# ysymyth/3D-SDN

Measured on AMD Instinct MI355X. Metric: rendered-objects/sec (FFD decode + transform + silhouette/normal/depth @384, fwd+bwd), higher is better.
Workload: dtype f32

## Files before the change

3d-sdn_amd/csrc/transform.hip:

```cpp
#include "sdn_common.h"

namespace sdn {

struct PtfParams {
    const float* verts;
    const float* scales;
    const float* quat;
    const float* trans;
    const float* persp;
    const float* zoom_to;
    const float* zoom_fixed;
    float* out;
    float* zooms;
    unsigned long long* key;
    int n, V;
};

__device__ __forceinline__ void quat_matrix(const float* q, float T[9])
{
    const float a = q[0], b = q[1], c = q[2], d = q[3];
    T[0] = ((a * a + b * b) - c * c) - d * d;
    T[1] = 2 * b * c - 2 * a * d;
    T[2] = 2 * b * d + 2 * a * c;
    T[3] = 2 * b * c + 2 * a * d;
// ... 42 lines not shown
    if (P.zoom_fixed) return;
#pragma unroll
    for (int o = 32; o > 0; o >>= 1) {
        const unsigned long long other = __shfl_xor(key, o, 64);
        key = other < key ? other : key;
    }
    if ((threadIdx.x & 63) == 0) red[threadIdx.x >> 6] = key;
    __syncthreads();
    if (threadIdx.x == 0) {
        unsigned long long k = red[0];
        for (int i = 1; i < 4; i++) k = red[i] < k ? red[i] : k;
        P.key[P.n + (size_t)b * gridDim.x + blockIdx.x] = k;
    }
}

__global__ __launch_bounds__(256) void k_ptf_fwd_b(const PtfParams P)
{
    __shared__ unsigned long long red[4];
    const int b = blockIdx.y;
    const int v = blockIdx.x * 256 + threadIdx.x;
    unsigned long long key = ~0ull;
    for (unsigned i = threadIdx.x; i < gridDim.x; i += 256) {
        const unsigned long long k = P.key[P.n + (size_t)b * gridDim.x + i];
        key = k < key ? k : key;
    }
#pragma unroll
    for (int o = 32; o > 0; o >>= 1) {
        const unsigned long long other = __shfl_xor(key, o, 64);
        key = other < key ? other : key;
    }
    if ((threadIdx.x & 63) == 0) red[threadIdx.x >> 6] = key;
    __syncthreads();
    key = red[0];
    for (int i = 1; i < 4; i++) key = red[i] < key ? red[i] : key;
    if (v >= P.V) return;
    const float zoom = __uint_as_float((unsigned)(key >> 32)) * P.zoom_to[b];
    float* o = P.out + ((size_t)b * P.V + v) * 3;
    o[2] = o[2] / zoom;
    if (v == 0) {
        P.zooms[b] = zoom;
        P.key[b] = key;
    }
}

struct PtfBwdParams {
    PtfParams f;
    const float* out;
    const float* g_out;
    const float* g_zooms;
    float* g_verts;
    float* acc;
    float* g_scales;
    float* g_quat;
    float* g_trans;
    float* g_persp;
    float* g_zoom_to;
    int s_parts;
};

__global__ __launch_bounds__(256) void k_ptf_bwd_a(const PtfBwdParams B)
{
    __shared__ float red[4];
    const int b = blockIdx.y, V = B.f.V;
    float s = 0.f;
    for (int v = blockIdx.x * 256 + threadIdx.x; v < V; v += gridDim.x * 256) {
        const size_t i = ((size_t)b * V + v) * 3 + 2;
        s += B.g_out[i] * B.out[i];
    }
#pragma unroll
    for (int o = 32; o > 0; o >>= 1) s += __shfl_xor(s, o, 64);
    if ((threadIdx.x & 63) == 0) red[threadIdx.x >> 6] = s;
    __syncthreads();
    if (threadIdx.x == 0) B.acc[20 * (size_t)B.f.n + 16 * b + blockIdx.x] = ((red[0] + red[1]) + red[2]) + red[3];
    if (blockIdx.x == 0 && threadIdx.x < 20) B.acc[20 * b + threadIdx.x] = 0.f;
}

__device__ __forceinline__ float ptf_S(const PtfBwdParams& B, int b, int nparts)
{
    float s = 0.f;
    for (int i = 0; i < nparts; i++) s += B.acc[20 * (size_t)B.f.n + 16 * b + i];
    return s;
}

__global__ __launch_bounds__(256) void k_ptf_bwd_b(const PtfBwdParams B)
{
    __shared__ float red[4][18];
    const int b = blockIdx.y, V = B.f.V;
    const int v = blockIdx.x * 256 + threadIdx.x;
    float part[18];
#pragma unroll
    for (int k = 0; k < 18; k++) part[k] = 0.f;
    if (v < V) {
        float T[9];
        quat_matrix(B.f.quat + 4 * b, T);
        const float* sc = B.f.scales + 3 * b;
        const float* p0 = B.f.persp + 3 * b;
        const unsigned long long key = B.f.key[b];
        const float rmin = __uint_as_float((unsigned)(key >> 32));
        const int vstar = (int)(unsigned)(key & 0xffffffffull);
        const float zoom = rmin * B.f.zoom_to[b];
        float dzoom = -ptf_S(B, b, B.s_parts) / zoom;
        if (B.g_zooms) dzoom += B.g_zooms[b];
        const size_t i = ((size_t)b * V + v) * 3;
        const float X = B.out[i], Y = B.out[i + 1], Z = B.out[i + 2] * zoom;
        float gX = B.g_out[i], gY = B.g_out[i + 1], gZ = B.g_out[i + 2] / zoom;
        if (v == vstar) {
            const float dr = dzoom * B.f.zoom_to[b];
            const float ax = fabsf(X), ay = fabsf(Y);
            const float m = fmaxf(ax, ay);
            gZ += dr * (Z >= 0.f ? 1.f : -1.f) / m;
            const float dm = -dr * fabsf(Z) / (m * m);
            if (ax >= ay)
                gX += dm * (X >= 0.f ? 1.f : -1.f);
            else
                gY += dm * (Y >= 0.f ? 1.f : -1.f);
        }
        const float kx = p0[0] / p0[2], ky = p0[1] / p0[2];
        const float gw0 = gX, gw1 = gY, gw2 = (gZ - kx * gX) - ky * gY;
        part[3] = -gX * Z / p0[2];
        part[4] = -gY * Z / p0[2];
        part[5] = (gX * p0[0] + gY * p0[1]) * Z / (p0[2] * p0[2]);
        part[0] = gw0;
        part[1] = gw1;
        part[2] = gw2;
        const float* vin = B.f.verts + i;
        const float u0 = vin[0] * sc[0], u1 = vin[1] * sc[1], u2 = vin[2] * sc[2];
        part[6] = gw0 * u0;
        part[7] = gw0 * u1;
        part[8] = gw0 * u2;
        part[9] = gw1 * u0;
        part[10] = gw1 * u1;
        part[11] = gw1 * u2;
        part[12] = gw2 * u0;
        part[13] = gw2 * u1;
        part[14] = gw2 * u2;
        const float gu0 = (T[0] * gw0 + T[3] * gw1) + T[6] * gw2;
        const float gu1 = (T[1] * gw0 + T[4] * gw1) + T[7] * gw2;
        const float gu2 = (T[2] * gw0 + T[5] * gw1) + T[8] * gw2;
        part[15] = gu0 * vin[0];
        part[16] = gu1 * vin[1];
        part[17] = gu2 * vin[2];
        float* gv = B.g_verts + i;
        gv[0] = gu0 * sc[0];
        gv[1] = gu1 * sc[1];
        gv[2] = gu2 * sc[2];
    }
#pragma unroll
    for (int k = 0; k < 18; k++) {
        float s = part[k];
#pragma unroll
        for (int o = 32; o > 0; o >>= 1) s += __shfl_xor(s, o, 64);
        if ((threadIdx.x & 63) == 0) red[threadIdx.x >> 6][k] = s;
    }
    __syncthreads();
    if (threadIdx.x < 18)
        unsafeAtomicAdd(B.acc + 20 * b + threadIdx.x,
                        ((red[0][threadIdx.x] + red[1][threadIdx.x]) + red[2][threadIdx.x]) + red[3][threadIdx.x]);
}

__global__ void k_ptf_bwd_c(const PtfBwdParams B)
{
    const int b = blockIdx.x * blockDim.x + threadIdx.x;
    if (b >= B.f.n) return;
    const float* A = B.acc + 20 * b;
    const float* q = B.f.quat + 4 * b;
    const float a = q[0], bq = q[1], c = q[2], d = q[3];
    const float* g = A + 6;
    B.g_quat[4 * b + 0] = 2 * a * ((g[0] + g[4]) + g[8]) + 2 * (((((-d * g[1] + c * g[2]) + d * g[3]) - bq * g[5]) - c * g[6]) + bq * g[7]);
    B.g_quat[4 * b + 1] = 2 * bq * ((g[0] - g[4]) - g[8]) + 2 * (((((c * g[1] + d * g[2]) + c * g[3]) - a * g[5]) + d * g[6]) + a * g[7]);
    B.g_quat[4 * b + 2] = 2 * c * ((-g[0] + g[4]) - g[8]) + 2 * (((((bq * g[1] + a * g[2]) + bq * g[3]) + d * g[5]) - a * g[6]) + d * g[7]);
    B.g_quat[4 * b + 3] = 2 * d * ((-g[0] - g[4]) + g[8]) + 2 * (((((-a * g[1] + bq * g[2]) + a * g[3]) + c * g[5]) + bq * g[6]) + c * g[7]);
    for (int k = 0; k < 3; k++) {
        if (B.g_persp == B.g_trans) {
            B.g_trans[3 * b + k] = A[k] + A[3 + k];
        } else {
            B.g_trans[3 * b + k] = A[k];
            B.g_persp[3 * b + k] = A[3 + k];
        }
        B.g_scales[3 * b + k] = A[15 + k];
    }
    const unsigned long long key = B.f.key[b];
    const float rmin = __uint_as_float((unsigned)(key >> 32));
    const float zoom = rmin * B.f.zoom_to[b];
    float dzoom = -ptf_S(B, b, B.s_parts) / zoom;
    if (B.g_zooms) dzoom += B.g_zooms[b];
    B.g_zoom_to[b] = dzoom * rmin;
}

}

using namespace sdn;

SDN_API int sdn_perspective_transform_scratch(int n, int V, size_t* key_bytes, size_t* acc_bytes)
{
    if (n <= 0 || V <= 0 || (!key_bytes && !acc_bytes))
        return fail(SDN_EINVAL, "sdn_perspective_transform_scratch: bad arguments");
    if (key_bytes) *key_bytes = (size_t)n * (1 + (size_t)cdiv(V, 256)) * sizeof(unsigned long long);
    if (acc_bytes) *acc_bytes = (size_t)n * 36 * sizeof(float);
    return SDN_OK;
}

SDN_API int sdn_perspective_transform(const float* verts, const float* scales, const float* quat, const float* trans,
                                      const float* persp, const float* zoom_to, const float* zoom_fixed, int n, int V,
                                      float* out, float* zooms, void* key, sdnStream stream)
{
    if (!verts || !scales || !quat || !trans || !persp || (!zoom_to && !zoom_fixed) || !out || !zooms || !key || n <= 0 ||
        V <= 0)
        return fail(SDN_EINVAL, "sdn_perspective_transform: bad arguments");
    hipStream_t st = (hipStream_t)stream;
    PtfParams P{verts, scales, quat, trans, persp, zoom_to, zoom_fixed, out, zooms, (unsigned long long*)key, n, V};
    const dim3 grid(cdiv(V, 256), (unsigned)n);
    if (zoom_fixed) {
        hipLaunchKernelGGL(k_ptf_fwd_a, grid, dim3(256), 0, st, P);
        return check_launch("k_ptf_fwd (given zoom)");
    }
    hipLaunchKernelGGL(k_ptf_fwd_a, grid, dim3(256), 0, st, P);
    hipLaunchKernelGGL(k_ptf_fwd_b, grid, dim3(256), 0, st, P);
    return check_launch("k_ptf_fwd");
}

SDN_API int sdn_perspective_transform_bwd(const float* verts, const float* scales, const float* quat, const float* trans,
                                          const float* persp, const float* zoom_to, int n, int V, const float* out,
                                          const void* key, const float* g_out, const float* g_zooms, float* g_verts,
                                          float* g_scales, float* g_quat, float* g_trans, float* g_persp,
                                          float* g_zoom_to, float* acc, sdnStream stream)
{
    if (!verts || !scales || !quat || !trans || !persp || !zoom_to || !out || !key || !g_out || !g_verts || !g_scales ||
        !g_quat || !g_trans || !g_persp || !g_zoom_to || !acc || n <= 0 || V <= 0)
        return fail(SDN_EINVAL, "sdn_perspective_transform_bwd: bad arguments");
    hipStream_t st = (hipStream_t)stream;
    PtfBwdParams B;
    B.f = PtfParams{verts, scales, quat, trans, persp, zoom_to, nullptr, nullptr, nullptr, (unsigned long long*)key, n, V};
    B.out = out;
    B.g_out = g_out;
    B.g_zooms = g_zooms;
    B.g_verts = g_verts;
    B.acc = acc;
    B.g_scales = g_scales;
    B.g_quat = g_quat;
    B.g_trans = g_trans;
    B.g_persp = g_persp;
    B.g_zoom_to = g_zoom_to;
    const unsigned vb = cdiv(V, 256);
    B.s_parts = (int)(vb < 16 ? vb : 16);
    hipLaunchKernelGGL(k_ptf_bwd_a, dim3((unsigned)B.s_parts, (unsigned)n), dim3(256), 0, st, B);
    hipLaunchKernelGGL(k_ptf_bwd_b, dim3(vb, (unsigned)n), dim3(256), 0, st, B);
    hipLaunchKernelGGL(k_ptf_bwd_c, dim3(cdiv(n, 64)), dim3(64), 0, st, B);
    return check_launch("k_ptf_bwd");
}

namespace sdn {

__global__ __launch_bounds__(64) void k_pose_params(const float* __restrict__ theta, const float* __restrict__ log_scales, int n,
                                                    float* __restrict__ quat, float* __restrict__ scales)
{
    const int i = blockIdx.x * 64 + threadIdx.x;
    if (i >= n) return;
    const float h = theta[i] / 2;
    quat[4 * i + 0] = cosf(h);
    quat[4 * i + 1] = 0.f;
    quat[4 * i + 2] = sinf(h);
    quat[4 * i + 3] = 0.f;
#pragma unroll
    for (int d = 0; d < 3; d++) scales[3 * i + d] = expf(log_scales[3 * i + d]);
}

__global__ __launch_bounds__(64) void k_pose_params_bwd(const float* __restrict__ theta, const float* __restrict__ scales,
                                                        const float* __restrict__ g_quat, const float* __restrict__ g_scales, int n,
                                                        float* __restrict__ g_theta, float* __restrict__ g_log_scales)
{
    const int i = blockIdx.x * 64 + threadIdx.x;
    if (i >= n) return;
    if (g_theta) {
        const float h = theta[i] / 2;
        const float a = g_quat ? g_quat[4 * i + 0] : 0.f, c = g_quat ? g_quat[4 * i + 2] : 0.f;
        g_theta[i] = (a * (-sinf(h)) + c * cosf(h)) / 2;
    }
    if (g_log_scales) {
#pragma unroll
        for (int d = 0; d < 3; d++) g_log_scales[3 * i + d] = g_scales ? g_scales[3 * i + d] * scales[3 * i + d] : 0.f;
    }
}

struct PoseAlgebra {
    const float *centre, *extent, *focals, *delta, *log_scales, *log_depths, *t2;
    float *theta, *alpha, *quat, *scales, *depth, *c2, *trans, *persp, *zoom;
    int n, training;
    float image_size, render_size;
};

__device__ __forceinline__ void camera_ray(float row, float col, float r[3], float* norm)
{
    const float l = sqrtf((col * col + row * row) + 1.0f);
    r[0] = col / l;
    r[1] = -row / l;
    r[2] = -1.0f / l;
    *norm = l;
}

__global__ __launch_bounds__(64) void k_pose_algebra(const PoseAlgebra P)
{
    const int i = blockIdx.x * 64 + threadIdx.x;
    if (i >= P.n) return;
    const float d0 = P.delta[2 * i], d1 = P.delta[2 * i + 1];
    const float theta = atan2f(d1, d0);
    P.theta[i] = theta;
    const float h = theta / 2;
    P.quat[4 * i + 0] = cosf(h);
    P.quat[4 * i + 1] = 0.f;
    P.quat[4 * i + 2] = sinf(h);
    P.quat[4 * i + 3] = 0.f;
#pragma unroll
    for (int d = 0; d < 3; d++) P.scales[3 * i + d] = expf(P.log_scales[3 * i + d]);
    const float e0 = P.extent[2 * i], e1 = P.extent[2 * i + 1], c0 = P.centre[2 * i], c1 = P.centre[2 * i + 1];
    const float depth = sqrtf(expf(P.log_depths[i]) / (e0 * e1));
    P.depth[i] = depth;
    const float q0 = c0 + P.t2[2 * i] * e0, q1 = c1 + P.t2[2 * i + 1] * e1;
    P.c2[2 * i] = q0;
    P.c2[2 * i + 1] = q1;
    float r[3], l;
    camera_ray(q0, q1, r, &l);
    const float tx = depth * r[0], ty = depth * r[1], tz = depth * r[2];
    P.trans[3 * i] = tx;
    P.trans[3 * i + 1] = ty;
    P.trans[3 * i + 2] = tz;
    const float a = -(theta - atanf(tx / tz)) + 3.14159265358979323846f;
    const float two_pi = 6.28318530717958647692f;
    float m = fmodf(a, two_pi);
    if (m != 0.f && m < 0.f) m += two_pi;
    P.alpha[i] = m - 3.14159265358979323846f;
// ... 130 lines not shown
```

3d-sdn_amd/csrc/raster_fwd.hip:

```cpp
#include <mutex>
#include <type_traits>
#include <vector>

#include "camera_math.h"
#include "raster_math.h"
#include "sdn_common.h"

namespace sdn {

constexpr int TS = 32;
constexpr int NTHR = (TS / 2) * (TS / 2);
constexpr int NWAVE = NTHR / 64;
static_assert(NTHR % 64 == 0 && NTHR >= 2 * TS && TS <= 32, "tile / workgroup geometry (hit queue packs px, py in 5 bits)");
constexpr int QCAP = 512;
constexpr int FREC = 13;
#ifndef SDN_LAB_SMALL_AREA
#define SDN_LAB_SMALL_AREA 32
#endif
constexpr int SMALL_AREA = SDN_LAB_SMALL_AREA;
#ifndef SDN_LAB_SPAN_AREA
#define SDN_LAB_SPAN_AREA 256
#endif
constexpr int SPAN_AREA = SDN_LAB_SPAN_AREA;
#ifndef SDN_LAB_HIZ_MIN_LIST
#define SDN_LAB_HIZ_MIN_LIST 257
#endif
constexpr int HIZ_MIN_LIST = SDN_LAB_HIZ_MIN_LIST;
#ifndef SDN_K1_HIZ
#define SDN_K1_HIZ 1
#endif
constexpr uint32_t TB_CULLED = 0x000000FFu;

struct FwdParams {
    const float* faces;
    const float* textures;
    const float* bg;
    float* face_inv;
    int32_t* face_index_map;
    float* weight_map;
    float* depth_map;
    float* rgb_map;
    float* rgb_out;
    float* alpha_out;
    float* depth_out;
    const uint32_t* tilebox;
    const uint4* pixbox;
    const uint32_t* tile_off;
    const uint32_t* tile_list;
    const uint32_t* overflow;
    const uint32_t* tile_order;
    const uint32_t* thin_count;
    const float4* thin_list;
    unsigned long long* counters;
    uint32_t list_cap;
    double eps;
    int ts, bs, nf, S, ntx, flags, bg_per_batch;
    int hiz;
    float near_le, far_f;
};

constexpr float THIN_MARGIN = 4.0f;

__device__ __forceinline__ float face_margin_px(const float f[9], int S)
{
    const float ex0 = f[3] - f[0], ey0 = f[4] - f[1];
    const float ex1 = f[6] - f[0], ey1 = f[7] - f[1];
    const float ex2 = f[6] - f[3], ey2 = f[7] - f[4];
    const float l0 = sqrtf(ex0 * ex0 + ey0 * ey0);
    const float l1 = sqrtf(ex1 * ex1 + ey1 * ey1);
    const float l2 = sqrtf(ex2 * ex2 + ey2 * ey2);
    const float lmax = fmaxf(l0, fmaxf(l1, l2));
    const float perim = l0 + l1 + l2;
    float cmax = fmaxf(fmaxf(fabsf(f[0]), fabsf(f[1])), fmaxf(fabsf(f[3]), fabsf(f[4])));
    cmax = fmaxf(cmax, fmaxf(fabsf(f[6]), fabsf(f[7])));
    const float area2 = fabsf(ex0 * ey1 - ex1 * ey0) - 9.5367432e-7f * lmax * lmax;
    if (!(area2 > 0.0f)) return -1.0f;
    const float delta = 9.5367432e-7f * (1.0f + cmax);
    const float base = 0.004f * fmaxf(1.0f, (float)S * (1.0f / 1024.0f)) + 0.5f * (float)S * delta;
    const float m = base + 0.5f * (float)S * (delta * perim * lmax / area2);
    if (!(m < (float)S)) return -1.0f;
    return m;
}

constexpr int HIST_MAX = 4096;

template <bool K1, bool GATHER>
__global__ __launch_bounds__(256) void k_face_setup(const float* __restrict__ faces, int nf, int S, int ntx,
                                                     float* __restrict__ face_inv, uint32_t* __restrict__ tilebox,
                                                     uint4* __restrict__ pixbox, uint32_t* __restrict__ tile_count,
                                                     uint32_t* __restrict__ thin_count, float4* __restrict__ thin_list,
                                                     const FaceSource G)
{
    __shared__ uint32_t hist[HIST_MAX];
    const int ntiles = ntx * ntx;
    const bool use_lds = ntiles <= HIST_MAX;
    if (use_lds)
        for (int t = threadIdx.x; t < ntiles; t += 256) hist[t] = 0u;
    __syncthreads();
    const int b = blockIdx.y;
    const int t_local = blockIdx.x * 256 + threadIdx.x;
    uint32_t* gcount = tile_count + (size_t)b * ntiles;
    const bool pairs = GATHER && G.fill_back != 0;
    const int nthr = pairs ? G.nf0 : nf;
    float v[3][3], pf[9];
    if constexpr (GATHER) {
        if (t_local < nthr) {
// ... 408 lines not shown
#pragma unroll
        for (int dx = 0; dx < 2; dx++) {
            const int dy = 1 - dyi;
            const int px = 2 * qx + dx, py = 2 * qy + dy;
            const int gx = X0 + px, gy = Y0 + py;
            if (gx >= S || gy >= S) continue;
            any_valid = true;
            const PixelResult r = shade_pixel(P, b, zbuf[py * TS + px], gx, gy);
            const size_t q = ((size_t)b * S + gy) * S + gx;
            if (save) {
                P.face_index_map[q] = r.fn;
                P.depth_map[q] = r.zp;
            }
            if (save && !lazy) {
                P.weight_map[q * 3 + 0] = r.w[0];
                P.weight_map[q * 3 + 1] = r.w[1];
                P.weight_map[q * 3 + 2] = r.w[2];
                if (want_rgb) {
                    P.rgb_map[q * 3 + 0] = r.rgb[0];
                    P.rgb_map[q * 3 + 1] = r.rgb[1];
                    P.rgb_map[q * 3 + 2] = r.rgb[2];
                }
            }
            if (aa) {
                s_alpha = s_alpha + r.alpha;
                s_depth = s_depth + r.zp;
#pragma unroll
                for (int k = 0; k < 3; k++) s_rgb[k] = s_rgb[k] + r.rgb[k];
            } else {
                const size_t o = ((size_t)b * S + (S - 1 - gy)) * S + gx;
                if (want_alpha) P.alpha_out[o] = r.alpha;
                if (want_depth) P.depth_out[o] = r.zp;
                if (want_rgb) {
#pragma unroll
                    for (int k = 0; k < 3; k++)
                        P.rgb_out[(((size_t)b * 3 + k) * S + (S - 1 - gy)) * S + gx] = r.rgb[k];
                }
            }
        }
    }
    if (aa && any_valid) {
        const int oc = X0 / 2 + qx;
        const int orow = R - 1 - (Y0 / 2 + qy);
        const size_t o = ((size_t)b * R + orow) * R + oc;
        if (want_alpha) P.alpha_out[o] = s_alpha * 0.25f;
        if (want_depth) P.depth_out[o] = s_depth * 0.25f;
        if (want_rgb) {
#pragma unroll
            for (int k = 0; k < 3; k++) P.rgb_out[(((size_t)b * 3 + k) * R + orow) * R + oc] = s_rgb[k] * 0.25f;
        }
    }
}

__device__ __forceinline__ void hiz_refresh(const uint32_t* zhi, uint32_t* blockmax, const int lane)
{
    uint32_t m[4] = {0u, 0u, 0u, 0u};
#pragma unroll
    for (int i = 0; i < 16; i++) m[i >> 2] = max(m[i >> 2], zhi[2 * (i * 64 + lane) + 1]);
#pragma unroll
    for (int rb = 0; rb < 4; rb++) {
        uint32_t v = m[rb];
        v = max(v, (uint32_t)__shfl_xor((int)v, 1, 64));
        v = max(v, (uint32_t)__shfl_xor((int)v, 2, 64));
        v = max(v, (uint32_t)__shfl_xor((int)v, 4, 64));
        v = max(v, (uint32_t)__shfl_xor((int)v, 32, 64));
        m[rb] = v;
    }
    if ((lane & 39) == 0) {
#pragma unroll
        for (int rb = 0; rb < 4; rb++) blockmax[rb * 4 + (lane >> 3)] = m[rb];
    }
    __builtin_amdgcn_wave_barrier();
}
__device__ __forceinline__ bool hiz_hidden(const uint32_t* blockmax, const uint32_t zc, const int x0, const int x1, const int y0,
                                           const int y1)
{
    uint32_t zb = 0u;
    for (int by = y0 >> 3; by <= (y1 >> 3); by++)
        for (int bx = x0 >> 3; bx <= (x1 >> 3); bx++) zb = max(zb, blockmax[by * (TS / 8) + bx]);
    return zc > zb;
}

template <bool COUNT, int HIZ>
__global__ __launch_bounds__(NTHR) void k_raster_tiles(const FwdParams P)
{
    unsigned n_cand = 0, n_in = 0, n_key = 0;
    unsigned long long c_fetch = 0, c_small = 0, c_large = 0, c_thin = 0, c_epi = 0, t_mark = 0, t_begin = 0;
    auto tick = [&](unsigned long long& acc) {
        if constexpr (COUNT) {
            const unsigned long long now = wall_clock64();
            acc += now - t_mark;
            t_mark = now;
        }
    };
    if constexpr (COUNT) t_begin = t_mark = wall_clock64();
    __shared__ unsigned long long zbuf[TS * TS];
    __shared__ uint32_t q_fn[QCAP];
    __shared__ float xtab[TS], ytab[TS];
    __shared__ uint32_t q_count, next_batch, next_thin;
    __shared__ uint32_t hit_queue[NWAVE][128];
    __shared__ float face_rec[NWAVE][64 * FREC];
    __shared__ uint32_t blockmax[(TS / 8) * (TS / 8)];
    static_assert(TS == 32, "the hi-z refresh maps 64 lanes x 16 reads onto a 32 x 32 tile");

    const int tid = threadIdx.x;
    const int lane = tid & 63, wave = tid >> 6;
    const int ntiles_all = P.ntx * P.ntx;
    const uint32_t gid = P.tile_order[blockIdx.x];
    const int b = (int)(gid / (uint32_t)ntiles_all), tile = (int)(gid % (uint32_t)ntiles_all);
    const int tx = tile % P.ntx, ty = tile / P.ntx;
    const int X0 = tx * TS, Y0 = ty * TS;
    const int S = P.S, nf = P.nf;

    for (int i = tid; i < TS * TS; i += NTHR) zbuf[i] = ~0ull;
    if (tid < TS)
        xtab[tid] = pixel_to_ndc(X0 + tid, S);
    else if (tid < 2 * TS)
        ytab[tid - TS] = pixel_to_ndc(Y0 + tid - TS, S);
    if (tid == 0) q_count = next_batch = next_thin = 0;
    if (tid < (TS / 8) * (TS / 8)) blockmax[tid] = 0xffffffffu;
    __syncthreads();

    const float4* thin_cull = P.thin_list + (size_t)b * nf * 2;
    const uint32_t n_thin = P.thin_count[b];
    const float4 thin_c0 = thin_cull[min(tid, 2 * nf - 1)];
    const uint32_t* tb = P.tilebox + (size_t)b * nf;
    const uint4* pbx = P.pixbox + (size_t)b * nf;
    const float* faces_b = P.faces + (size_t)b * nf * 9;
    const float* finv_b = P.face_inv + (size_t)b * nf * 9;

    auto shade_hit = [&](const float z0, const float z1, const float z2, const float (&inv)[9], const uint32_t qf,
                         const int px, const int py) {
        float bw[3];
        bary_weights(inv, X0 + px, Y0 + py, bw);
        const float zp = persp_depth(bw, z0, z1, z2);
        if (zp > P.near_le && zp < P.far_f) {
            if constexpr (COUNT) n_key++;
            const unsigned long long key = ((unsigned long long)ord_bits(zp) << 32) | qf;
            atomicMin(&zbuf[py * TS + px], key);
        }
    };
    uint32_t* hq = hit_queue[wave];
    float* frec = face_rec[wave];
    int hq_n = 0;
    auto drain = [&](const int count) {
        if (lane < count) {
            const uint32_t e = hq[lane];
            const int slot = (int)(e & 63u), px = (int)((e >> 6) & 31u), py = (int)((e >> 11) & 31u);
            const float* r = frec + slot * FREC;
            float inv[9];
#pragma unroll
            for (int k = 0; k < 9; k++) inv[k] = r[3 + k];
            shade_hit(r[0], r[1], r[2], inv, __float_as_uint(r[12]), px, py);
        }
    };
    const uint32_t* zhi = reinterpret_cast<const uint32_t*>(zbuf);
    auto behind = [&](const uint32_t zc, const int px, const int py) -> bool { return zc > zhi[2 * (py * TS + px) + 1]; };
    bool hiz_on = false;
    auto refresh_hiz = [&]() { hiz_refresh(zhi, blockmax, lane); };
    auto push_hits = [&](const bool hit, const uint32_t entry) {
        const unsigned long long hm = __ballot(hit);
        if (hm) {
            if (hit) hq[hq_n + (int)__popcll(hm & ((1ull << lane) - 1ull))] = entry;
            hq_n += (int)__popcll(hm);
            __builtin_amdgcn_wave_barrier();
            if (hq_n >= 64) {
                drain(64);
                __builtin_amdgcn_wave_barrier();
                const uint32_t rest = (lane < hq_n - 64) ? hq[64 + lane] : 0u;
                __builtin_amdgcn_wave_barrier();
                hq[lane] = rest;
                hq_n -= 64;
                __builtin_amdgcn_wave_barrier();
            }
        }
    };
    auto raster_batch = [&](const uint32_t* ids, const int n) {
        if constexpr (HIZ > 0) {
            if (HIZ == 1 || hiz_on) refresh_hiz();
        }
        const int kshift = 31 - __clz(64 / n);
        const int k = 1 << kshift;
        const int q = lane >> kshift, sub = lane & (k - 1);
        const bool mine = q < n;
        const uint32_t qf_l = mine ? ids[q] : 0u;
        uint4 pb_l = make_uint4(0u, 0u, 0u, 0u);
        float f_l[9], inv_l[9];
#pragma unroll
        for (int kk = 0; kk < 9; kk++) f_l[kk] = inv_l[kk] = 0.0f;
        if (mine) {
            pb_l = pbx[qf_l];
#pragma unroll
            for (int kk = 0; kk < 9; kk++) f_l[kk] = faces_b[(size_t)qf_l * 9 + kk];
#pragma unroll
            for (int kk = 0; kk < 9; kk++) inv_l[kk] = finv_b[(size_t)qf_l * 9 + kk];
        }
        const int lx0 = max((int)(pb_l.x & 0xffffu), X0), lx1 = min((int)(pb_l.x >> 16), X0 + TS - 1);
        const int ly0 = max((int)(pb_l.y & 0xffffu), Y0), ly1 = min((int)(pb_l.y >> 16), Y0 + TS - 1);
        const int lw = lx1 - lx0 + 1, lh = ly1 - ly0 + 1;
        int area_l = (mine && lw > 0 && lh > 0) ? lw * lh : 0;
        const float zmin_l = fminf(f_l[2], fminf(f_l[5], f_l[8]));
        const uint32_t zc_l = (zmin_l > 0.0f) ? ord_bits(zmin_l * 0.99999f) : 0u;
        if constexpr (HIZ > 0) {
            if ((HIZ == 1 || hiz_on) && area_l > 0 && zc_l != 0u && hiz_hidden(blockmax, zc_l, lx0 - X0, lx1 - X0, ly0 - Y0, ly1 - Y0))
                area_l = 0;
        }
        if (mine && sub == 0) {
            float* r = frec + q * FREC;
            r[0] = f_l[2];
            r[1] = f_l[5];
            r[2] = f_l[8];
#pragma unroll
            for (int kk = 0; kk < 9; kk++) r[3 + kk] = inv_l[kk];
            r[12] = __uint_as_float(qf_l);
        }
        __builtin_amdgcn_wave_barrier();
        if constexpr (COUNT) {
            asm volatile("s_waitcnt vmcnt(0) lgkmcnt(0)" ::: "memory");
            tick(c_fetch);
        }
        {
            const bool small = area_l > 0 && area_l <= SMALL_AREA * k;
            const float rw = 1.0f / (float)(lw > 0 ? lw : 1);
            for (int i = sub; __ballot(small && i < area_l) != 0ull; i += k) {
                bool hit = false;
                int px = 0, py = 0;
                if (small && i < area_l) {
                    const int yy = (int)(((float)i + 0.5f) * rw);
                    const int xx = i - yy * lw;
                    px = lx0 - X0 + xx;
                    py = ly0 - Y0 + yy;
                    if constexpr (COUNT) n_cand++;
                    hit = inside_ndc(f_l, xtab[px], ytab[py]);
                    if constexpr (COUNT) n_in += hit ? 1u : 0u;
                    if (hit) hit = !behind(zc_l, px, py);
                }
                push_hits(hit, (uint32_t)q | ((uint32_t)px << 6) | ((uint32_t)py << 11));
            }
        }
        tick(c_small);
        unsigned long long big = __ballot(area_l > SMALL_AREA * k && sub == 0);
        const float fS = (float)S, fS1 = (float)(S - 1);
        while (big) {
            const int j = __builtin_amdgcn_readfirstlane(__ffsll((long long)big) - 1);
            big &= big - 1ull;
            const int x0 = __builtin_amdgcn_readlane(lx0, j), y0 = __builtin_amdgcn_readlane(ly0, j);
            const int w = __builtin_amdgcn_readlane(lw, j), h = __builtin_amdgcn_readlane(lh, j);
            const uint32_t zc = (uint32_t)__builtin_amdgcn_readlane((int)zc_l, j);
            const float mj = __int_as_float(__builtin_amdgcn_readlane((int)pb_l.z, j));
            const uint32_t slot = (uint32_t)(j >> kshift);
            float f[9];
#pragma unroll
            for (int kk = 0; kk < 9; kk++) f[kk] = __int_as_float(__builtin_amdgcn_readlane(__float_as_int(f_l[kk]), j));
            if (w * h <= SPAN_AREA) {
                const int area = w * h;
                const float rw = 1.0f / (float)w;
                for (int i0 = 0; i0 < area; i0 += 64) {
                    const int i = i0 + lane;
                    bool hit = false;
                    int px = 0, py = 0;
                    if (i < area) {
                        const int yy = (int)(((float)i + 0.5f) * rw);
                        const int xx = i - yy * w;
                        px = x0 - X0 + xx;
                        py = y0 - Y0 + yy;
                        if constexpr (COUNT) n_cand++;
                        hit = inside_ndc(f, xtab[px], ytab[py]);
                        if constexpr (COUNT) n_in += hit ? 1u : 0u;
                        if (hit) hit = !behind(zc, px, py);
                    }
                    push_hits(hit, slot | ((uint32_t)px << 6) | ((uint32_t)py << 11));
                }
                continue;
            }
            const int hs = h > 1 ? 32 - __clz(h - 1) : 0;
            const int rshift = 6 - hs, per_row = 1 << rshift;
            const int row = lane >> rshift, rsub = lane & (per_row - 1);
            const bool rvalid = row < h;
            const int py = y0 - Y0 + (rvalid ? row : 0);
            const float yp = ytab[py];
            const int bx0 = x0 - X0;
            float lo = (float)bx0, hi = (float)(bx0 + w - 1);
#pragma unroll
            for (int e = 0; e < 3; e++) {
                const float xa = f[3 * e], ya = f[3 * e + 1], xb = f[(3 * e + 3) % 9], yb = f[(3 * e + 4) % 9];
                const float D = xb - xa, E = yb - ya;
                if (E != 0.0f) {
                    const float rE = __builtin_amdgcn_rcpf(E);
                    const float xe = xa + (yp - ya) * D * rE;
                    const float pe = (xe * fS + fS1) * 0.5f - (float)X0;
                    const float sl = mj * __builtin_amdgcn_sqrtf(D * D + E * E) * fabsf(rE) + 1.0f;
                    if (E > 0.0f)
                        hi = fminf(hi, pe + sl);
                    else
                        lo = fmaxf(lo, pe - sl);
                }
            }
            const int xl = max(bx0, (int)floorf(fminf(lo, 64.0f)));
            const int xr = min(bx0 + w - 1, (int)ceilf(fmaxf(hi, -64.0f)));
            const int len = rvalid ? xr - xl + 1 : 0;
            for (int i = rsub; __ballot(i < len) != 0ull; i += per_row) {
                bool hit = false;
                int px = 0;
                if (i < len) {
                    px = xl + i;
                    if constexpr (COUNT) n_cand++;
                    hit = inside_ndc(f, xtab[px], yp);
                    if constexpr (COUNT) n_in += hit ? 1u : 0u;
                    if (hit) hit = !behind(zc, px, py);
                }
                push_hits(hit, slot | ((uint32_t)px << 6) | ((uint32_t)py << 11));
            }
        }
        if (hq_n) {
            drain(hq_n);
            hq_n = 0;
            __builtin_amdgcn_wave_barrier();
        }
        tick(c_large);
    };

    const float4* thin_recs = thin_cull + nf;
    auto thin_cull_pass = [&]() {
        const float cx = (float)X0 + 0.5f * (float)(TS - 1), cy = (float)Y0 + 0.5f * (float)(TS - 1);
        const float reach = 0.7072f * (float)TS + 0.4f;
#ifndef SDN_LAB_NO_THIN_CULL
        for (uint32_t t = tid; t < n_thin; t += NTHR) {
            const float4 c = t < (uint32_t)NTHR ? thin_c0 : thin_cull[t];
            if (fabsf(cx * c.x + cy * c.y - c.z) > c.w + reach) continue;
            const uint32_t slot = atomicAdd(&q_count, 1u);
            if (slot < (uint32_t)QCAP) q_fn[slot] = t;
        }
#endif
    };
    auto thin_items = [&]() {
#ifndef SDN_LAB_NO_THIN
        const uint32_t queued = q_count;
        const bool all = queued > (uint32_t)QCAP;
        const uint32_t n_loop = all ? n_thin : queued;
        constexpr int ROWS_PER_ITEM = 8, GROUPS = TS / ROWS_PER_ITEM;
        for (;;) {
            uint32_t first = 0;
            if (lane == 0) first = atomicAdd(&next_thin, 64u);
            first = (uint32_t)__builtin_amdgcn_readfirstlane((int)first);
            if (first >= n_loop * GROUPS) break;
            const uint32_t item = first + (uint32_t)lane;
            if (item >= n_loop * GROUPS) continue;
            const uint32_t c = item / GROUPS;
            const int g = (int)(item % GROUPS);
            const uint32_t t = all ? c : q_fn[c];
            const float4 e0 = thin_cull[t], e1 = thin_recs[t];
            const float nx = e0.x, ny = e0.y, band = e0.w, ax = e1.x, ay = e1.y;
            const uint32_t qf = __float_as_uint(e1.z);
            float f[9];
            bool loaded = false;
            for (int py = g * ROWS_PER_ITEM; py < (g + 1) * ROWS_PER_ITEM; py++) {
                const float off = ((float)(Y0 + py) - ay) * ny;
// ... 720 lines not shown
```

Before: 23570.

## Fuse perspective-transform backward finalize into main kernel via last-block ticket

Merges the per-object finalize kernel into the main backward kernel: the last block to arrive for each object, detected with an atomic ticket counter in slot 19 of the accumulator, computes the quaternion, translation, scale and zoom gradients. The main kernel also becomes a grid-stride loop with 1024-thread blocks capped at 16 blocks per object, so each thread accumulates several vertices in registers before one batched shuffle reduction. This removes a kernel launch and cuts the number of atomics, in exchange for release/acquire fence handling and fewer, larger blocks. The ticket counter relies on slot 19 being zeroed by the earlier kernel, which it is.

```diff
diff --git a/3d-sdn_amd/csrc/transform.hip b/3d-sdn_amd/csrc/transform.hip
--- a/3d-sdn_amd/csrc/transform.hip
+++ b/3d-sdn_amd/csrc/transform.hip
@@ -148,87 +148,20 @@
     return s;
 }
 
-__global__ __launch_bounds__(256) void k_ptf_bwd_b(const PtfBwdParams B)
-{
-    __shared__ float red[4][18];
-    const int b = blockIdx.y, V = B.f.V;
-    const int v = blockIdx.x * 256 + threadIdx.x;
-    float part[18];
-#pragma unroll
-    for (int k = 0; k < 18; k++) part[k] = 0.f;
-    if (v < V) {
-        float T[9];
-        quat_matrix(B.f.quat + 4 * b, T);
-        const float* sc = B.f.scales + 3 * b;
-        const float* p0 = B.f.persp + 3 * b;
-        const unsigned long long key = B.f.key[b];
-        const float rmin = __uint_as_float((unsigned)(key >> 32));
-        const int vstar = (int)(unsigned)(key & 0xffffffffull);
-        const float zoom = rmin * B.f.zoom_to[b];
-        float dzoom = -ptf_S(B, b, B.s_parts) / zoom;
-        if (B.g_zooms) dzoom += B.g_zooms[b];
-        const size_t i = ((size_t)b * V + v) * 3;
-        const float X = B.out[i], Y = B.out[i + 1], Z = B.out[i + 2] * zoom;
-        float gX = B.g_out[i], gY = B.g_out[i + 1], gZ = B.g_out[i + 2] / zoom;
-        if (v == vstar) {
-            const float dr = dzoom * B.f.zoom_to[b];
-            const float ax = fabsf(X), ay = fabsf(Y);
-            const float m = fmaxf(ax, ay);
-            gZ += dr * (Z >= 0.f ? 1.f : -1.f) / m;
-            const float dm = -dr * fabsf(Z) / (m * m);
-            if (ax >= ay)
-                gX += dm * (X >= 0.f ? 1.f : -1.f);
-            else
-                gY += dm * (Y >= 0.f ? 1.f : -1.f);
-        }
-        const float kx = p0[0] / p0[2], ky = p0[1] / p0[2];
-        const float gw0 = gX, gw1 = gY, gw2 = (gZ - kx * gX) - ky * gY;
-        part[3] = -gX * Z / p0[2];
-        part[4] = -gY * Z / p0[2];
-        part[5] = (gX * p0[0] + gY * p0[1]) * Z / (p0[2] * p0[2]);
-        part[0] = gw0;
-        part[1] = gw1;
-        part[2] = gw2;
-        const float* vin = B.f.verts + i;
-        const float u0 = vin[0] * sc[0], u1 = vin[1] * sc[1], u2 = vin[2] * sc[2];
-        part[6] = gw0 * u0;
-        part[7] = gw0 * u1;
-        part[8] = gw0 * u2;
-        part[9] = gw1 * u0;
-        part[10] = gw1 * u1;
-        part[11] = gw1 * u2;
-        part[12] = gw2 * u0;
-        part[13] = gw2 * u1;
-        part[14] = gw2 * u2;
-        const float gu0 = (T[0] * gw0 + T[3] * gw1) + T[6] * gw2;
-        const float gu1 = (T[1] * gw0 + T[4] * gw1) + T[7] * gw2;
-        const float gu2 = (T[2] * gw0 + T[5] * gw1) + T[8] * gw2;
-        part[15] = gu0 * vin[0];
-        part[16] = gu1 * vin[1];
-        part[17] = gu2 * vin[2];
-        float* gv = B.g_verts + i;
-        gv[0] = gu0 * sc[0];
-        gv[1] = gu1 * sc[1];
-        gv[2] = gu2 * sc[2];
-    }
-#pragma unroll
-    for (int k = 0; k < 18; k++) {
-        float s = part[k];
-#pragma unroll
-        for (int o = 32; o > 0; o >>= 1) s += __shfl_xor(s, o, 64);
-        if ((threadIdx.x & 63) == 0) red[threadIdx.x >> 6][k] = s;
-    }
-    __syncthreads();
-    if (threadIdx.x < 18)
-        unsafeAtomicAdd(B.acc + 20 * b + threadIdx.x,
-                        ((red[0][threadIdx.x] + red[1][threadIdx.x]) + red[2][threadIdx.x]) + red[3][threadIdx.x]);
-}
-
-__global__ void k_ptf_bwd_c(const PtfBwdParams B)
-{
-    const int b = blockIdx.x * blockDim.x + threadIdx.x;
-    if (b >= B.f.n) return;
-    const float* A = B.acc + 20 * b;
+#ifdef SDN_LAB_PTF_G
+constexpr int PTF_BWD_G = SDN_LAB_PTF_G;
+#else
+constexpr int PTF_BWD_G = 16;
+#endif
+#ifdef SDN_LAB_PTF_THREADS
+constexpr int PTF_BWD_NT = SDN_LAB_PTF_THREADS;
+#else
+constexpr int PTF_BWD_NT = 1024;
+#endif
+constexpr int PTF_TICKET = 19;
+
+__device__ __forceinline__ void ptf_finish(const PtfBwdParams& B, int b, const float* A)
+{
     const float* q = B.f.quat + 4 * b;
     const float a = q[0], bq = q[1], c = q[2], d = q[3];
     const float* g = A + 6;
@@ -251,6 +184,104 @@
     float dzoom = -ptf_S(B, b, B.s_parts) / zoom;
     if (B.g_zooms) dzoom += B.g_zooms[b];
     B.g_zoom_to[b] = dzoom * rmin;
+}
+
+__global__ __launch_bounds__(PTF_BWD_NT) void k_ptf_bwd_b(const PtfBwdParams B)
+{
+    constexpr int NT = PTF_BWD_NT, NW = NT / 64;
+    __shared__ float red[NW][18];
+    const int b = blockIdx.y, V = B.f.V;
+    float part[18];
+#pragma unroll
+    for (int k = 0; k < 18; k++) part[k] = 0.f;
+    float T[9];
+    quat_matrix(B.f.quat + 4 * b, T);
+    const float sc0 = B.f.scales[3 * b], sc1 = B.f.scales[3 * b + 1], sc2 = B.f.scales[3 * b + 2];
+    const float p00 = B.f.persp[3 * b], p01 = B.f.persp[3 * b + 1], p02 = B.f.persp[3 * b + 2];
+    const unsigned long long key = B.f.key[b];
+    const float rmin = __uint_as_float((unsigned)(key >> 32));
+    const int vstar = (int)(unsigned)(key & 0xffffffffull);
+    const float zoom_to = B.f.zoom_to[b];
+    const float zoom = rmin * zoom_to;
+    float dzoom = -ptf_S(B, b, B.s_parts) / zoom;
+    if (B.g_zooms) dzoom += B.g_zooms[b];
+    const float kx = p00 / p02, ky = p01 / p02;
+    for (int v = blockIdx.x * NT + threadIdx.x; v < V; v += gridDim.x * NT) {
+        const size_t i = ((size_t)b * V + v) * 3;
+        const float X = B.out[i], Y = B.out[i + 1], Z = B.out[i + 2] * zoom;
+        float gX = B.g_out[i], gY = B.g_out[i + 1], gZ = B.g_out[i + 2] / zoom;
+        if (v == vstar) {
+            const float dr = dzoom * zoom_to;
+            const float ax = fabsf(X), ay = fabsf(Y);
+            const float m = fmaxf(ax, ay);
+            gZ += dr * (Z >= 0.f ? 1.f : -1.f) / m;
+            const float dm = -dr * fabsf(Z) / (m * m);
+            if (ax >= ay)
+                gX += dm * (X >= 0.f ? 1.f : -1.f);
+            else
+                gY += dm * (Y >= 0.f ? 1.f : -1.f);
+        }
+        const float gw0 = gX, gw1 = gY, gw2 = (gZ - kx * gX) - ky * gY;
+        part[3] += -gX * Z / p02;
+        part[4] += -gY * Z / p02;
+        part[5] += (gX * p00 + gY * p01) * Z / (p02 * p02);
+        part[0] += gw0;
+        part[1] += gw1;
+        part[2] += gw2;
+        const float* vin = B.f.verts + i;
+        const float vin0 = vin[0], vin1 = vin[1], vin2 = vin[2];
+        const float u0 = vin0 * sc0, u1 = vin1 * sc1, u2 = vin2 * sc2;
+        part[6] += gw0 * u0;
+        part[7] += gw0 * u1;
+        part[8] += gw0 * u2;
+        part[9] += gw1 * u0;
+        part[10] += gw1 * u1;
+        part[11] += gw1 * u2;
+        part[12] += gw2 * u0;
+        part[13] += gw2 * u1;
+        part[14] += gw2 * u2;
+        const float gu0 = (T[0] * gw0 + T[3] * gw1) + T[6] * gw2;
+        const float gu1 = (T[1] * gw0 + T[4] * gw1) + T[7] * gw2;
+        const float gu2 = (T[2] * gw0 + T[5] * gw1) + T[8] * gw2;
+        part[15] += gu0 * vin0;
+        part[16] += gu1 * vin1;
+        part[17] += gu2 * vin2;
+        float* gv = B.g_verts + i;
+        gv[0] = gu0 * sc0;
+        gv[1] = gu1 * sc1;
+        gv[2] = gu2 * sc2;
+    }
+#pragma unroll
+    for (int o = 32; o > 0; o >>= 1) {
+        float other[18];
+#pragma unroll
+        for (int k = 0; k < 18; k++) other[k] = __shfl_xor(part[k], o, 64);
+#pragma unroll
+        for (int k = 0; k < 18; k++) part[k] += other[k];
+    }
+    if ((threadIdx.x & 63) == 0) {
+#pragma unroll
+        for (int k = 0; k < 18; k++) red[threadIdx.x >> 6][k] = part[k];
+    }
+    __syncthreads();
+    if (threadIdx.x < 18) {
+        float s = red[0][threadIdx.x];
+        for (int w = 1; w < NW; w++) s += red[w][threadIdx.x];
+#ifndef SDN_LAB_PTF_NO_ATOMICS
+        unsafeAtomicAdd(B.acc + 20 * b + threadIdx.x, s);
+#endif
+        __builtin_amdgcn_fence(__ATOMIC_RELEASE, "agent");
+        asm volatile("s_waitcnt vmcnt(0)" ::: "memory");
+    }
+    __syncthreads();
+    if (threadIdx.x != 0) return;
+    unsigned* ticket = reinterpret_cast<unsigned*>(B.acc + 20 * b + PTF_TICKET);
+    if (__hip_atomic_fetch_add(ticket, 1u, __ATOMIC_RELAXED, __HIP_MEMORY_SCOPE_AGENT) != gridDim.x - 1) return;
+    __builtin_amdgcn_fence(__ATOMIC_ACQUIRE, "wavefront");
+    float A[18];
+#pragma unroll
+    for (int k = 0; k < 18; k++) A[k] = __hip_atomic_load(B.acc + 20 * b + k, __ATOMIC_RELAXED, __HIP_MEMORY_SCOPE_AGENT);
+    ptf_finish(B, b, A);
 }
 
 }
@@ -307,11 +338,10 @@
     B.g_trans = g_trans;
     B.g_persp = g_persp;
     B.g_zoom_to = g_zoom_to;
-    const unsigned vb = cdiv(V, 256);
+    const unsigned vb = cdiv(V, 256), vg = cdiv(V, PTF_BWD_NT);
     B.s_parts = (int)(vb < 16 ? vb : 16);
     hipLaunchKernelGGL(k_ptf_bwd_a, dim3((unsigned)B.s_parts, (unsigned)n), dim3(256), 0, st, B);
-    hipLaunchKernelGGL(k_ptf_bwd_b, dim3(vb, (unsigned)n), dim3(256), 0, st, B);
-    hipLaunchKernelGGL(k_ptf_bwd_c, dim3(cdiv(n, 64)), dim3(64), 0, st, B);
+    hipLaunchKernelGGL(k_ptf_bwd_b, dim3(vg < (unsigned)PTF_BWD_G ? vg : (unsigned)PTF_BWD_G, (unsigned)n), dim3(PTF_BWD_NT), 0, st, B);
     return check_launch("k_ptf_bwd");
 }
 
```

Measured after the change: 23550 (median of 2 runs). No clear change (-0.1%).

## Flatten small and mid-size face pixel candidates into a compacted wave-wide stream

Applied to the files above, without the earlier changes.

Replaces the per-face sub-lane split for small faces and the per-face span loop for mid-size faces with a single flattened candidate stream. A prefix scan over each face's bounding-box area gives every lane one candidate pixel per pass, and the owning face is found through an LDS start-mark strip plus ds_permute/bpermute. Faces above FLAT_MAX still go to the row-based large path. The aim is to remove the idle lanes of per-face loops, at the cost of extra cross-lane shuffles per pass. The launch bounds also gain an occupancy hint of 6.

```diff
diff --git a/3d-sdn_amd/csrc/raster_fwd.hip b/3d-sdn_amd/csrc/raster_fwd.hip
--- a/3d-sdn_amd/csrc/raster_fwd.hip
+++ b/3d-sdn_amd/csrc/raster_fwd.hip
@@ -14,14 +14,11 @@
 static_assert(NTHR % 64 == 0 && NTHR >= 2 * TS && TS <= 32, "tile / workgroup geometry (hit queue packs px, py in 5 bits)");
 constexpr int QCAP = 512;
 constexpr int FREC = 13;
-#ifndef SDN_LAB_SMALL_AREA
-#define SDN_LAB_SMALL_AREA 32
+#ifndef SDN_LAB_FLAT_MAX
+#define SDN_LAB_FLAT_MAX 256
 #endif
-constexpr int SMALL_AREA = SDN_LAB_SMALL_AREA;
-#ifndef SDN_LAB_SPAN_AREA
-#define SDN_LAB_SPAN_AREA 256
-#endif
-constexpr int SPAN_AREA = SDN_LAB_SPAN_AREA;
+constexpr int FLAT_MAX = SDN_LAB_FLAT_MAX;
+static_assert(FLAT_MAX >= 1 && FLAT_MAX <= 256, "a batch's stream holds at most 64 * 256 candidates: 14 bits of start, at most 256 passes (the marks are u16, 0xffff = none)");
 #ifndef SDN_LAB_HIZ_MIN_LIST
 #define SDN_LAB_HIZ_MIN_LIST 257
 #endif
@@ -596,7 +593,7 @@
 }
 
 template <bool COUNT, int HIZ>
-__global__ __launch_bounds__(NTHR) void k_raster_tiles(const FwdParams P)
+__global__ __launch_bounds__(NTHR, 6) void k_raster_tiles(const FwdParams P)
 {
     unsigned n_cand = 0, n_in = 0, n_key = 0;
     unsigned long long c_fetch = 0, c_small = 0, c_large = 0, c_thin = 0, c_epi = 0, t_mark = 0, t_begin = 0;
@@ -615,6 +612,7 @@
     __shared__ uint32_t hit_queue[NWAVE][128];
     __shared__ float face_rec[NWAVE][64 * FREC];
     __shared__ uint32_t blockmax[(TS / 8) * (TS / 8)];
+    __shared__ uint32_t own_strip[NWAVE][32];
     static_assert(TS == 32, "the hi-z refresh maps 64 lanes x 16 reads onto a 32 x 32 tile");
 
     const int tid = threadIdx.x;
@@ -693,11 +691,8 @@
         if constexpr (HIZ > 0) {
             if (HIZ == 1 || hiz_on) refresh_hiz();
         }
-        const int kshift = 31 - __clz(64 / n);
-        const int k = 1 << kshift;
-        const int q = lane >> kshift, sub = lane & (k - 1);
-        const bool mine = q < n;
-        const uint32_t qf_l = mine ? ids[q] : 0u;
+        const bool mine = lane < n;
+        const uint32_t qf_l = mine ? ids[lane] : 0u;
         uint4 pb_l = make_uint4(0u, 0u, 0u, 0u);
         float f_l[9], inv_l[9];
 #pragma unroll
@@ -719,8 +714,8 @@
             if ((HIZ == 1 || hiz_on) && area_l > 0 && zc_l != 0u && hiz_hidden(blockmax, zc_l, lx0 - X0, lx1 - X0, ly0 - Y0, ly1 - Y0))
                 area_l = 0;
         }
-        if (mine && sub == 0) {
-            float* r = frec + q * FREC;
+        if (mine) {
+            float* r = frec + lane * FREC;
             r[0] = f_l[2];
             r[1] = f_l[5];
             r[2] = f_l[8];
@@ -733,60 +728,77 @@
             asm volatile("s_waitcnt vmcnt(0) lgkmcnt(0)" ::: "memory");
             tick(c_fetch);
         }
+        unsigned long long big = __ballot(area_l > FLAT_MAX);
         {
-            const bool small = area_l > 0 && area_l <= SMALL_AREA * k;
-            const float rw = 1.0f / (float)(lw > 0 ? lw : 1);
-            for (int i = sub; __ballot(small && i < area_l) != 0ull; i += k) {
+            const int fa = area_l <= FLAT_MAX ? area_l : 0;
+            int incl = fa;
+#pragma unroll
+            for (int d = 1; d < 64; d <<= 1) {
+                const int o = __shfl_up(incl, d, 64);
+                if (lane >= d) incl += o;
+            }
+            const int T = __builtin_amdgcn_readlane(incl, 63);
+            const int box_l = ((lx0 - X0) & 31) | (((ly0 - Y0) & 31) << 5) | (((lw - 1) & 31) << 10) | ((incl - fa) << 15) |
+                              (fa > 0 ? 0 : (int)0x80000000);
+            const float rw_l = 1.0f / (float)(lw > 0 ? lw : 1);
+            const unsigned long long fm = __ballot(fa > 0);
+            const int below = (int)__builtin_amdgcn_mbcnt_hi((uint32_t)(fm >> 32), __builtin_amdgcn_mbcnt_lo((uint32_t)fm, 0u));
+            const int rank_l = fa > 0 ? below : (int)__popcll(fm) + lane - below;
+            const int lane_of_rank = __builtin_amdgcn_ds_permute(rank_l << 2, lane);
+            uint32_t* strip = own_strip[wave];
+            uint16_t* strip16 = reinterpret_cast<uint16_t*>(strip);
+            if (lane < 32) strip[lane] = 0xffffffffu;
+            __builtin_amdgcn_wave_barrier();
+            int rank0 = -1;
+            for (int base = 0, pass = 0; base < T; base += 64, pass++) {
+                const int rel = (box_l >> 15) - base;
+                if ((unsigned)rel < 64u) strip16[rel] = (uint16_t)pass;
+                __builtin_amdgcn_wave_barrier();
+                const bool starts = (int)strip16[lane] == pass;
+                __builtin_amdgcn_wave_barrier();
+                const unsigned long long sm = __ballot(starts);
+                const int rk = (int)__builtin_amdgcn_mbcnt_hi((uint32_t)(sm >> 32),
+                                                              __builtin_amdgcn_mbcnt_lo((uint32_t)sm, (uint32_t)(rank0 + (starts ? 1 : 0))));
+                rank0 += (int)__popcll(sm);
+                const int s = __builtin_amdgcn_ds_bpermute(rk << 2, lane_of_rank);
+                const int a4 = s << 2;
+                const int box = __builtin_amdgcn_ds_bpermute(a4, box_l);
+                const float rw = __int_as_float(__builtin_amdgcn_ds_bpermute(a4, __float_as_int(rw_l)));
+                const uint32_t zc = (uint32_t)__builtin_amdgcn_ds_bpermute(a4, (int)zc_l);
+                float f[9];
+#pragma unroll
+                for (int kk = 0; kk < 9; kk++)
+                    f[kk] = (kk % 3 == 2) ? 0.0f : __int_as_float(__builtin_amdgcn_ds_bpermute(a4, __float_as_int(f_l[kk])));
                 bool hit = false;
                 int px = 0, py = 0;
-                if (small && i < area_l) {
+                if (base + lane < T) {
+                    const int i = base + lane - (box >> 15);
                     const int yy = (int)(((float)i + 0.5f) * rw);
-                    const int xx = i - yy * lw;
-                    px = lx0 - X0 + xx;
-                    py = ly0 - Y0 + yy;
+                    const int xx = i - yy * (((box >> 10) & 31) + 1);
+                    px = (box & 31) + xx;
+                    py = ((box >> 5) & 31) + yy;
                     if constexpr (COUNT) n_cand++;
-                    hit = inside_ndc(f_l, xtab[px], ytab[py]);
+                    hit = inside_ndc(f, xtab[px], ytab[py]);
                     if constexpr (COUNT) n_in += hit ? 1u : 0u;
-                    if (hit) hit = !behind(zc_l, px, py);
+                    if (hit) hit = !behind(zc, px, py);
                 }
-                push_hits(hit, (uint32_t)q | ((uint32_t)px << 6) | ((uint32_t)py << 11));
+                push_hits(hit, (uint32_t)s | ((uint32_t)px << 6) | ((uint32_t)py << 11));
             }
         }
         tick(c_small);
-        unsigned long long big = __ballot(area_l > SMALL_AREA * k && sub == 0);
         const float fS = (float)S, fS1 = (float)(S - 1);
         while (big) {
             const int j = __builtin_amdgcn_readfirstlane(__ffsll((long long)big) - 1);
             big &= big - 1ull;
-            const int x0 = __builtin_amdgcn_readlane(lx0, j), y0 = __builtin_amdgcn_readlane(ly0, j);
-            const int w = __builtin_amdgcn_readlane(lw, j), h = __builtin_amdgcn_readlane(lh, j);
+            const uint32_t pbx_j = (uint32_t)__builtin_amdgcn_readlane((int)pb_l.x, j), pby_j = (uint32_t)__builtin_amdgcn_readlane((int)pb_l.y, j);
+            const int x0 = max((int)(pbx_j & 0xffffu), X0), y0 = max((int)(pby_j & 0xffffu), Y0);
+            const int w = min((int)(pbx_j >> 16), X0 + TS - 1) - x0 + 1, h = min((int)(pby_j >> 16), Y0 + TS - 1) - y0 + 1;
             const uint32_t zc = (uint32_t)__builtin_amdgcn_readlane((int)zc_l, j);
             const float mj = __int_as_float(__builtin_amdgcn_readlane((int)pb_l.z, j));
-            const uint32_t slot = (uint32_t)(j >> kshift);
+            const uint32_t slot = (uint32_t)j;
             float f[9];
 #pragma unroll
             for (int kk = 0; kk < 9; kk++) f[kk] = __int_as_float(__builtin_amdgcn_readlane(__float_as_int(f_l[kk]), j));
-            if (w * h <= SPAN_AREA) {
-                const int area = w * h;
-                const float rw = 1.0f / (float)w;
-                for (int i0 = 0; i0 < area; i0 += 64) {
-                    const int i = i0 + lane;
-                    bool hit = false;
-                    int px = 0, py = 0;
-                    if (i < area) {
-                        const int yy = (int)(((float)i + 0.5f) * rw);
-                        const int xx = i - yy * w;
-                        px = x0 - X0 + xx;
-                        py = y0 - Y0 + yy;
-                        if constexpr (COUNT) n_cand++;
-                        hit = inside_ndc(f, xtab[px], ytab[py]);
-                        if constexpr (COUNT) n_in += hit ? 1u : 0u;
-                        if (hit) hit = !behind(zc, px, py);
-                    }
-                    push_hits(hit, slot | ((uint32_t)px << 6) | ((uint32_t)py << 11));
-                }
-                continue;
-            }
             const int hs = h > 1 ? 32 - __clz(h - 1) : 0;
             const int rshift = 6 - hs, per_row = 1 << rshift;
             const int row = lane >> rshift, rsub = lane & (per_row - 1);
```

Result: faster. 23520 before, 24020 after (median of 6 runs) (+2.1%).
